# QuasarX1/astro-sph-tools

Hardware: AMD Instinct MI355X
Metric: Mpixels/s + particles/s, 10^8-particle 4096² projection at 1/2/4/8 MI355X (higher is better)
Workload: dtype f32; 1 GPU; cfg3: 1e+08 particles -> 4096^2 mass-weighted temperature map, wendland_c2, pixel-scale h, fp32; particles=100000000, grid=4096, kernel=wendland_c2, h_law=pixel, map=weighted, parallelism=single, accumulation=fp64, collective_overlap=False, streams=1, scatter_gate=False

## Files before the change

astro-sph-tools_amd/csrc/asp_device.hpp:

```cpp
#pragma once

#include <hip/hip_runtime.h>
#include <stdint.h>

namespace asp {

constexpr int kBlock = 256;
#ifndef ASP_DEP_BLOCK
#define ASP_DEP_BLOCK 512
#endif
constexpr int kDepBlock = ASP_DEP_BLOCK;
constexpr int kTile = 64;
constexpr int kTileShift = 6;
constexpr int kRow = kTile + 1;
constexpr int kTileWords = kTile * kRow;
constexpr int kWideTilesDefault = 256;
constexpr int kScaleBits = 49;
constexpr int kAccF64 = 0;
constexpr int kAccFix = 1;

struct Grid {
    double x_min, y_min;
    double psx;
    double psy_pix;
    double psy_cull;
    float xminf, yminf;
    float ipsx, ipsy;
    float mg;
    float mgl;
    int nx, ny, cs;
    int gnx;
    int ox;
    int ncx, ncy;
    int ntx, nty, ntiles;
    int nonsquare;
    int mixed;
    int wide_tiles;
    int gather_min;
    int gather_area;
};

struct Src64 {
    const double* u64;
    const double* v64;
    const double* cu64;
    const double* cv64;
    const double* h64;
    long long stride;
    const float* u32;
    const float* v32;
    const float* h32;
};

struct Box {
    int x0, x1, y0, y1;
};

struct Prep {
    float u, v, h;
    float lo;
    float hi;
    float hinv;
    float s0, s1;
    float thr;
    float band;
    int p;
    Box b;
};

struct Item {
    long long start;
    int tile;
    int count;
    int slab;
    int mode;
};

struct Merge {
    int tile;
    int slab0;
    int nslab;
    int pad;
};

__device__ __forceinline__ double corner_x(const Grid& g, int xi) {
    return g.x_min + (double)(xi + g.ox) * g.psx;
}
__device__ __forceinline__ double corner_y(const Grid& g, int yi) {
    return g.y_min + (double)yi * g.psy_pix;
}

__device__ __forceinline__ bool cull_pass(const Grid& g, double u, double v, double h,
                                          int xi, int yi) {
    xi += g.ox;
    int xi0 = (xi / g.cs) * g.cs, yi0 = (yi / g.cs) * g.cs;
    int xe = min(xi0 + g.cs, g.gnx), ye = min(yi0 + g.cs, g.ny);
    double h2 = 2.0 * h;
    double xlo = g.x_min + (double)xi0 * g.psx, xhi = g.x_min + (double)xe * g.psx;
    double ylo = g.y_min + (double)yi0 * g.psy_cull, yhi = g.y_min + (double)ye * g.psy_cull;
    return (u >= xlo - h2) && (u < xhi + h2) && (v >= ylo - h2) && (v < yhi + h2);
}

__device__ __forceinline__ void chunk_range(double w, double h, double w_min, double ps,
                                            int npx, int cs, int& c_lo, int& c_hi) {
    int nc = (npx + cs - 1) / cs;
    double h2 = 2.0 * h;
    c_lo = 0;
    c_hi = -1;
    if (!__builtin_isfinite(w) || !__builtin_isfinite(h)) return;
    auto lo_ok = [&](int c) { return w >= (w_min + (double)(c * cs) * ps) - h2; };
    auto hi_ok = [&](int c) {
        int e = min((c + 1) * cs, npx);
        return w < (w_min + (double)e * ps) + h2;
    };
    double est = floor((w + h2 - w_min) / ((double)cs * ps));
    int cmax = est < -1.0 ? -1 : (est > nc - 1.0 ? nc - 1 : (int)est);
    while (cmax >= 0 && !lo_ok(cmax)) --cmax;
    while (cmax + 1 <= nc - 1 && lo_ok(cmax + 1)) ++cmax;
    double est2 = ceil((w - h2 - w_min) / ((double)cs * ps)) - 1.0;
    int cmin = est2 < 0.0 ? 0 : (est2 > (double)nc ? nc : (int)est2);
    while (cmin <= nc - 1 && !hi_ok(cmin)) ++cmin;
    while (cmin - 1 >= 0 && hi_ok(cmin - 1)) --cmin;
    c_lo = cmin;
    c_hi = cmax;
}

struct Vals {
    double U, V, CU, CV, H;
};
__device__ __forceinline__ Vals src_values(const Grid& g, const Src64& s, int p) {
    Vals r;
    if (s.u64) {
        const long long o = (long long)p * s.stride;
        r.U = s.u64[o];
        r.V = s.v64[o];
        r.H = s.h64[p];
        r.CU = g.mixed ? s.cu64[o] : r.U;
        r.CV = g.mixed ? s.cv64[o] : r.V;
    } else {
        r.U = r.CU = s.u32[p];
        r.V = r.CV = s.v32[p];
        r.H = s.h32[p];
    }
    return r;
}
__device__ __forceinline__ double src_u(const Src64& s, int p, float u) {
    return s.u64 ? s.u64[(long long)p * s.stride] : (double)u;
}
__device__ __forceinline__ double src_v(const Src64& s, int p, float v) {
    return s.v64 ? s.v64[(long long)p * s.stride] : (double)v;
}

template <bool CULL = true>
__device__ __forceinline__ bool footprint(const Grid& g, const Src64& s, int p, float u, float v,
                                          float h, Box& b) {
    float hd = fabsf(2.0f * h);
    if (!(hd > 0.0f) || !__builtin_isfinite(hd)) {
        return false;
    }
    if (!__builtin_isfinite(u) || !__builtin_isfinite(v)) return false;
    float cx = (u - g.xminf) * g.ipsx, rx = hd * g.ipsx;
    float cy = (v - g.yminf) * g.ipsy, ry = hd * g.ipsy;
    float dx = (fabsf(u) + fabsf(g.xminf) + hd) * g.ipsx * 0x1p-20f + 0x1p-12f;
    float dy = (fabsf(v) + fabsf(g.yminf) + hd) * g.ipsy * 0x1p-20f + 0x1p-12f;
    float fx0 = fmaxf(ceilf(cx - rx - dx), (float)g.ox);
    float fx1 = fminf(floorf(cx + rx + dx), (float)(g.ox + g.nx - 1));
    float fy0 = fmaxf(ceilf(cy - ry - dy), 0.0f);
    float fy1 = fminf(floorf(cy + ry + dy), (float)(g.ny - 1));
    if (!(fx0 <= fx1) || !(fy0 <= fy1)) return false;
    b.x0 = (int)fx0 - g.ox;
    b.x1 = (int)fx1 - g.ox;
    b.y0 = (int)fy0;
    b.y1 = (int)fy1;
    if (CULL && (g.nonsquare || g.mixed)) {
        const Vals x = src_values(g, s, p);
        int c0, c1;
        chunk_range(x.CV, x.H, g.y_min, g.psy_cull, g.ny, g.cs, c0, c1);
        b.y0 = max(b.y0, c0 * g.cs);
        b.y1 = min(b.y1, min((c1 + 1) * g.cs, g.ny) - 1);
        if (b.y0 > b.y1) return false;
        if (g.mixed) {
            chunk_range(x.CU, x.H, g.x_min, g.psx, g.gnx, g.cs, c0, c1);
            b.x0 = max(b.x0, c0 * g.cs - g.ox);
            b.x1 = min(b.x1, min((c1 + 1) * g.cs, g.gnx) - 1 - g.ox);
            if (b.x0 > b.x1) return false;
        }
    }
    return true;
}

template <int KID>
__device__ __forceinline__ double kernel_norm64(float h) {
    double hd = (double)h;
    double h3 = hd * hd * hd;
    double r = __builtin_amdgcn_rcp(h3);
    r = r * (2.0 - h3 * r);
    if constexpr (KID == 0) return (1.0 / M_PI) * r;
    else if constexpr (KID == 1) return (21.0 / (16.0 * M_PI)) * r;
    else return 1.0;
}

template <int KID>
__device__ __forceinline__ double term_coef(float a, float h) {
    return (double)a * kernel_norm64<KID>(h);
}

template <int KID>
__device__ __forceinline__ float kernel_shape(float q) {
    if constexpr (KID == 0) {
        float q2 = q * q;
        float a = fmaf(q2, fmaf(0.75f, q, -1.5f), 1.0f);
        float t = 2.0f - q;
        float b = 0.25f * (t * t * t);
        return q < 1.0f ? a : (q < 2.0f ? b : 0.0f);
    } else if constexpr (KID == 1) {
        float t = fmaxf(fmaf(-0.5f, q, 1.0f), 0.0f);
        float t2 = t * t;
        return (t2 * t2) * fmaf(2.0f, q, 1.0f);
    } else {
        return 1.0f;
    }
}

__device__ __forceinline__ float rec_thr(float h) {
    float D = 2.0f * h;
    return D * D;
}
__device__ __forceinline__ float rec_band(float mg, float h) {
    float Da = fabsf(2.0f * h);
    float eps = 0x1p-21f * (mg + Da);
    float band = 4.0f * Da * eps + 2.0f * eps * eps + 0x1p-20f * Da * Da;
    if (h < 0.0f || !__builtin_isfinite(band)) band = __builtin_inff();
    return band;
}

__device__ __forceinline__ void set_band(Prep& P, float thr, float band) {
    P.lo = thr - band;
    P.hi = thr + band;
    P.thr = thr;
    P.band = band;
}

template <int KID, int ACC = kAccF64>
__device__ __forceinline__ bool prep_record(const Grid& g, const Src64& s, int p, float u,
                                            float v, float h, float a0, float a1, int k0,
                                            int k1, Prep& P) {
    if (!footprint(g, s, p, u, v, h, P.b)) return false;
    P.u = u;
    P.v = v;
    P.h = h;
    P.p = p;
    set_band(P, rec_thr(h), rec_band(g.mg, h));
    P.hinv = __builtin_amdgcn_rcpf(h);
    if constexpr (ACC == kAccFix) {
        P.s0 = (float)ldexp(term_coef<KID>(a0, h), k0);
        P.s1 = (float)ldexp(term_coef<KID>(a1, h), k1);
    } else {
        P.s0 = (float)term_coef<KID>(a0, h);
        P.s1 = (float)term_coef<KID>(a1, h);
    }
    return true;
}

__device__ __forceinline__ bool exact_pair(const Grid& g, const Src64& s, int p, int xi, int yi) {
    const Vals x = src_values(g, s, p);
    double dx = x.U - corner_x(g, xi);
    double dy = x.V - corner_y(g, yi);
    double r2 = dx * dx + dy * dy;
    double t = 2.0 * x.H;
    return (r2 < t * t) && cull_pass(g, x.CU, x.CV, x.H, xi, yi);
}

__device__ __forceinline__ bool decide(const Grid& g, const Src64& s, const Prep& P, int xi,
                                       int yi, float X, float Y, float& r2) {
    float dx = P.u - X;
    float dy = P.v - Y;
    r2 = dx * dx + dy * dy;
    bool in = r2 < P.lo;
    if (r2 >= P.lo && r2 <= P.hi) in = exact_pair(g, s, P.p, xi, yi);
    return in;
}

__device__ __forceinline__ unsigned long long f2fix(float f) {
    const double magic = 6755399441055744.0;
    return (unsigned long long)(__double_as_longlong((double)f + magic) -
                                __double_as_longlong(magic));
}

template <int ACC>
__device__ __forceinline__ void acc_add(unsigned long long* a, float t) {
    if constexpr (ACC == kAccFix)
        atomicAdd(a, f2fix(t));
    else
        atomicAdd((double*)a, (double)t);
}

template <int ACC>
__device__ __forceinline__ float acc_value(unsigned long long s, int k) {
    if constexpr (ACC == kAccFix)
        return (float)ldexp((double)(long long)s, -k);
    else
        return (float)__longlong_as_double((long long)s);
}

template <int ACC>
__device__ __forceinline__ unsigned long long acc_sum(unsigned long long a, unsigned long long b) {
    if constexpr (ACC == kAccFix)
        return a + b;
    else
        return (unsigned long long)__double_as_longlong(__longlong_as_double((long long)a) +
                                                        __longlong_as_double((long long)b));
}

__device__ __forceinline__ float bcast(float x, int lane) {
// ... 51 lines not shown
```

astro-sph-tools_amd/csrc/asp_project2d.hip:

```cpp
#include <hip/hip_runtime.h>

#include <algorithm>
#include <cmath>
#include <cstdint>
#include <cstdio>
#include <cstdlib>
#include <cstring>
#include <mutex>
#include <string>
#include <type_traits>
#include <vector>

#include "../../include/asp.h"
#include "asp_binning.hpp"
#include "asp_device.hpp"
#include "asp_host.hpp"

namespace asp {

constexpr int kCountBlock = 256;
#ifndef ASP_COUNT_UNROLL
#define ASP_COUNT_UNROLL 4
#endif
constexpr int kCountUnroll = ASP_COUNT_UNROLL;
// ... 697 lines not shown
    if (idx < 0) return;
    float4 r0, r1;
    load_rec(recs, start + idx, r0, r1);
    Prep P;
    rec_prep<ACC>(r0, r1, X0, Y0, kk, P);
    if constexpr (EXT) ext_coef(P, ext[start + idx], pass);
    small_box<KID, NOUT, ACC, 4>(g, s, P, P.b.x1 - P.b.x0 + 1, P.b.y1 - P.b.y0 + 1, X0, Y0, xt,
                                 yt, acc0, acc1);
}

constexpr int kGatherThreads = 64;
constexpr int kGatherRegions = 8;
constexpr int kGatherPix = 8 * kGatherThreads;
static_assert(kGatherRegions * kGatherPix == kTile * kTile, "8 regions x 512 pixels cover the tile");
constexpr int kKernelIndicator = ASP_KERNEL_INDICATOR;
struct GEntry {
    float u, v, lo, hi, hinv, s0, s1;
    int p;
    unsigned box;
};
constexpr unsigned kNoBox = 0x00ff00ffu;

template <int NOUT, int ACC>
struct GAcc {
    unsigned long long a0[8], a1[8];
    f2 p0[4], p1[4];
    double* t0;
    double* t1;
    __device__ __forceinline__ void init(double* tot) {
#pragma unroll
        for (int j = 0; j < 8; ++j) {
            a0[j] = 0;
            a1[j] = 0;
        }
#pragma unroll
        for (int k = 0; k < 4; ++k) {
            p0[k] = (f2){0.0f, 0.0f};
            p1[k] = (f2){0.0f, 0.0f};
        }
        t0 = tot + threadIdx.x;
        t1 = tot + kGatherPix + threadIdx.x;
        if constexpr (ACC != kAccFix) {
#pragma unroll
            for (int j = 0; j < 8; ++j) {
                t0[j * kGatherThreads] = 0.0;
                if (NOUT == 2) t1[j * kGatherThreads] = 0.0;
            }
        }
    }
    __device__ __forceinline__ void add(int j, float w, float s0, float s1) {
        if constexpr (ACC == kAccFix) {
            a0[j] += f2fix(s0 * w);
            if (NOUT == 2) a1[j] += f2fix(s1 * w);
        } else {
            p0[j >> 1][j & 1] = fmaf(s0, w, p0[j >> 1][j & 1]);
            if (NOUT == 2) p1[j >> 1][j & 1] = fmaf(s1, w, p1[j >> 1][j & 1]);
        }
    }
    __device__ __forceinline__ void add2(int k, f2 w, float s0, float s1) {
        if constexpr (ACC == kAccFix) {
            add(2 * k, w.x, s0, s1);
            add(2 * k + 1, w.y, s0, s1);
        } else {
            p0[k] = __builtin_elementwise_fma(w, (f2){s0, s0}, p0[k]);
            if (NOUT == 2) p1[k] = __builtin_elementwise_fma(w, (f2){s1, s1}, p1[k]);
        }
    }
    __device__ __forceinline__ void fold() {
        if constexpr (ACC != kAccFix) {
#pragma unroll
            for (int j = 0; j < 8; ++j) {
                t0[j * kGatherThreads] += (double)p0[j >> 1][j & 1];
                if (NOUT == 2) t1[j * kGatherThreads] += (double)p1[j >> 1][j & 1];
            }
#pragma unroll
            for (int k = 0; k < 4; ++k) {
                p0[k] = (f2){0.0f, 0.0f};
                p1[k] = (f2){0.0f, 0.0f};
            }
        }
    }
    __device__ __forceinline__ unsigned long long word0(int j) const {
        if constexpr (ACC == kAccFix) return a0[j];
        else return (unsigned long long)__double_as_longlong(t0[j * kGatherThreads]);
    }
    __device__ __forceinline__ unsigned long long word1(int j) const {
        if constexpr (ACC == kAccFix) return a1[j];
        else return (unsigned long long)__double_as_longlong(t1[j * kGatherThreads]);
    }
};

template <int NOUT, int ACC>
constexpr size_t gather_lds() {
    return ACC == kAccFix ? 8 : (size_t)NOUT * kGatherPix * 8;
}

struct GOwn {
    int r0, c0;
    int lr, lc;
    __device__ __forceinline__ int row(int j) const { return r0 + 8 * (j >> 2) + lr; }
    __device__ __forceinline__ int col(int j) const { return c0 + 8 * (j & 3) + lc; }
};
__device__ __forceinline__ GOwn gather_owner(int w) {
    const int lane = threadIdx.x;
    GOwn o;
    o.r0 = (w >> 1) * 16;
    o.c0 = (w & 1) * 32;
    o.lr = lane >> 3;
    o.lc = lane & 7;
    return o;
}

__device__ __forceinline__ float corner_off_x(const Grid& g, int k) { return (float)((double)k * g.psx); }
__device__ __forceinline__ float corner_off_y(const Grid& g, int k) { return (float)((double)k * g.psy_pix); }

struct GCorner {
    float X[2], Y[4];
    float xl[2], xh[2], yl[2], yh[2];
};
__device__ __forceinline__ GCorner gather_corners(const Grid& g, const GOwn& o) {
    GCorner c;
    c.X[0] = corner_off_x(g, o.row(0));
    c.X[1] = corner_off_x(g, o.row(4));
#pragma unroll
    for (int k = 0; k < 4; ++k) c.Y[k] = corner_off_y(g, o.col(k));
#pragma unroll
    for (int r = 0; r < 2; ++r) {
        c.xl[r] = corner_off_x(g, o.r0 + 8 * r);
        c.xh[r] = corner_off_x(g, o.r0 + 8 * r + 7);
        c.yl[r] = corner_off_y(g, o.c0 + 16 * r);
        c.yh[r] = corner_off_y(g, o.c0 + 16 * r + 15);
    }
    return c;
}

__device__ __forceinline__ unsigned edge_mask(const GCorner& c, float u, float v, float thr) {
    float dx2[2], dy2[2];
#pragma unroll
    for (int r = 0; r < 2; ++r) {
        const float dx = u - fminf(fmaxf(u, c.xl[r]), c.xh[r]);
        const float dy = v - fminf(fmaxf(v, c.yl[r]), c.yh[r]);
        dx2[r] = dx * dx;
        dy2[r] = dy * dy;
    }
    const float lim = thr * (1.0f + 0x1p-8f);
    unsigned m = 0u;
#pragma unroll
    for (int r = 0; r < 2; ++r)
#pragma unroll
        for (int k = 0; k < 2; ++k) m |= (dx2[r] + dy2[k] < lim) ? 1u << (2 * r + k) : 0u;
    return m;
}

__device__ __forceinline__ GEntry make_gentry(const Prep& P, int X0, int Y0, float scale) {
    GEntry e;
    e.u = P.u; e.v = P.v; e.lo = P.lo; e.hi = P.hi; e.hinv = P.hinv;
    e.s0 = P.s0 * scale; e.s1 = P.s1 * scale; e.p = P.p;
    e.box = (unsigned)(P.b.x0 - X0) | ((unsigned)(P.b.x1 - X0) << 8) |
            ((unsigned)(P.b.y0 - Y0) << 16) | ((unsigned)(P.b.y1 - Y0) << 24);
    return e;
}

__device__ __forceinline__ bool meets_region(unsigned box, const GOwn& o) {
    return (int)(box & 255u) <= o.r0 + 15 && (int)((box >> 8) & 255u) >= o.r0 &&
           (int)((box >> 16) & 255u) <= o.c0 + 31 && (int)(box >> 24) >= o.c0;
}

__device__ __forceinline__ GEntry lane_entry(const GEntry& e, int l) {
    GEntry E;
    E.u = bcast(e.u, l); E.v = bcast(e.v, l); E.lo = bcast(e.lo, l); E.hi = bcast(e.hi, l);
    E.hinv = bcast(e.hinv, l); E.s0 = bcast(e.s0, l); E.s1 = bcast(e.s1, l);
    E.p = bcast(e.p, l); E.box = (unsigned)bcast((int)e.box, l);
    return E;
}

__device__ __forceinline__ unsigned block_hits(unsigned box, const GOwn& o) {
    const int x0 = box & 255u, x1 = (box >> 8) & 255u;
    const int y0 = (box >> 16) & 255u, y1 = box >> 24;
    unsigned m = 0u;
#pragma unroll
    for (int j = 0; j < 8; ++j) {
        const int br = o.r0 + 8 * (j >> 2), bc = o.c0 + 8 * (j & 3);
        if (x0 <= br + 7 && x1 >= br && y0 <= bc + 7 && y1 >= bc) m |= 1u << j;
    }
    return m;
}


template <int KID, int NOUT, int ACC>
__device__ __forceinline__ void gather_entry(const Grid& g, const Src64& s, const GEntry& E,
                                             int X0, int Y0, const GOwn& o, const GCorner& c,
                                             GAcc<NOUT, ACC>& ga) {
    const unsigned m = block_hits(E.box, o);
    const int x0 = E.box & 255u, x1 = (E.box >> 8) & 255u;
    const int y0 = (E.box >> 16) & 255u, y1 = E.box >> 24;
    unsigned in = 0u, amb = 0u;
#pragma unroll
    for (int j = 0; j < 8; ++j) {
        if (m & (1u << j)) {
            const float dx = E.u - c.X[j >> 2], dy = E.v - c.Y[j & 3];
            const float r2 = dx * dx + dy * dy;
            const bool inb = (unsigned)(o.row(j) - x0) <= (unsigned)(x1 - x0) &&
                             (unsigned)(o.col(j) - y0) <= (unsigned)(y1 - y0);
            in |= (inb && r2 < E.lo) ? (1u << j) : 0u;
            amb |= (inb && r2 >= E.lo && r2 <= E.hi) ? (1u << j) : 0u;
        }
    }
    for (unsigned a = amb; a; a &= a - 1u) {
        const int j = __builtin_ctz(a);
        if (exact_pair(g, s, E.p, X0 + o.row(j), Y0 + o.col(j))) in |= 1u << j;
    }
    const float sc = 1.0f / kShapeScale<KID>;
#pragma unroll
    for (int j = 0; j < 8; ++j) {
        if (in & (1u << j)) {
            const float dx = E.u - c.X[j >> 2], dy = E.v - c.Y[j & 3];
            const float r2 = dx * dx + dy * dy;
            const float wk = kernel_shape<KID>(__builtin_amdgcn_sqrtf(r2) * E.hinv) * sc;
            ga.add(j, wk, E.s0, E.s1);
        }
    }
}

template <int KID, int NOUT, int ACC>
__device__ __forceinline__ void gather_entry_masked(float u, float vs, float hinv, float s0,
                                                    float s1, float nt2, unsigned bm,
                                                    const GCorner& c, GAcc<NOUT, ACC>& ga) {
    const f2 hv = {-hinv, -hinv};
    const f2 dead = {nt2, nt2};
    const f2 vv = {vs, vs};
#pragma unroll
    for (int r = 0; r < 2; ++r) {
        if (bm & (3u << (2 * r))) {
            const float dxs = (u - c.X[r]) * hinv;
            const f2 dx2 = {dxs * dxs, dxs * dxs};
#pragma unroll
            for (int k = 0; k < 2; ++k) {
                if (bm & (1u << (2 * r + k))) {
                    const f2 dys = __builtin_elementwise_fma(hv, (f2){c.Y[2 * k], c.Y[2 * k + 1]}, vv);
                    const f2 r2 = __builtin_elementwise_fma(dys, dys, dx2);
                    f2 q;
                    q.x = __builtin_amdgcn_sqrtf(r2.x);
                    q.y = __builtin_amdgcn_sqrtf(r2.y);
                    ga.add2(2 * r + k, edge_shape2<KID, true>(q, dead), s0, s1);
                }
            }
        }
    }
}

template <int KID, int NOUT, int ACC>
__device__ __forceinline__ void gather_walk(const Grid& g, const Src64& s, const GEntry& mine,
                                            int X0, int Y0, const GOwn& o, const GCorner& c,
                                            GAcc<NOUT, ACC>& ga) {
    if (KID != kKernelIndicator && !g.nonsquare && !g.mixed) {
        const unsigned em = mine.box == kNoBox ? 0u : edge_mask(c, mine.u, mine.v, mine.hi);
        const float vs = mine.v * mine.hinv;
        const unsigned emd = em | (__float_as_uint(edge_dead2(mine.lo, mine.hi)) & ~15u);
        unsigned long long m = __ballot(em != 0u);
        while (m) {
            const int l = __builtin_ctzll(m);
            m &= m - 1;
            const unsigned w = (unsigned)bcast((int)emd, l);
            gather_entry_masked<KID, NOUT, ACC>(bcast(mine.u, l), bcast(vs, l), bcast(mine.hinv, l),
                                                bcast(mine.s0, l), bcast(mine.s1, l),
                                                __uint_as_float(w), w & 15u, c, ga);
        }
    } else {
        unsigned long long m = __ballot(meets_region(mine.box, o));
        while (m) {
            const int l = __builtin_ctzll(m);
            m &= m - 1;
            gather_entry<KID, NOUT, ACC>(g, s, lane_entry(mine, l), X0, Y0, o, c, ga);
        }
    }
    ga.fold();
}

template <int NOUT, int ACC>
__device__ __forceinline__ void gather_emit(const Grid& g, const GAcc<NOUT, ACC>& ga,
                                            const GOwn& o, int X0, int Y0, int slab,
                                            unsigned long long* slabs, int k0, int k1,
                                            float* out0, float* out1, int flags) {
    if (slab >= 0) {
        unsigned long long* dst = slabs + (long long)slab * NOUT * kTilePix;
#pragma unroll
        for (int j = 0; j < 8; ++j) {
            const int k = o.row(j) * kTile + o.col(j);
            dst[k] = ga.word0(j);
            if (NOUT == 2) dst[kTilePix + k] = ga.word1(j);
        }
        return;
    }
    const int TW = min(kTile, g.nx - X0), TH = min(kTile, g.ny - Y0);
#pragma unroll
    for (int j = 0; j < 8; ++j) {
        if (o.row(j) >= TW || o.col(j) >= TH) continue;
        const long long off = (long long)(X0 + o.row(j)) * g.ny + (Y0 + o.col(j));
        emit_pixel<NOUT, ACC>(off, ga.word0(j), NOUT == 2 ? ga.word1(j) : 0ull, k0, k1, out0,
                              out1, flags);
    }
}

__device__ __forceinline__ bool is_small(int bw, int bh) { return bw <= 4 && bh <= 4; }

template <int NOUT>
constexpr size_t deposit_lds() {
    return (size_t)NOUT * kTileWords * 8 + 2 * kTile * 4;
}

template <int KID, int NOUT, int ACC, int EXT = 0>
__global__ __launch_bounds__(kDepBlock) __attribute__((amdgpu_waves_per_eu(4))) void k_deposit(
    Grid g, Src64 s, const float4* __restrict__ recs, const Item* __restrict__ items,
    const int* __restrict__ order, const int2* __restrict__ tile_k,
    unsigned long long* __restrict__ slabs, float* __restrict__ out0, float* __restrict__ out1,
    int flags, const float4* __restrict__ ext, int pass) {
    extern __shared__ __attribute__((aligned(16))) unsigned long long acc[];
    unsigned long long* acc0 = acc;
    unsigned long long* acc1 = acc + kTileWords;
    float* xt = (float*)(acc + NOUT * kTileWords);
    float* yt = xt + kTile;
    __shared__ int defer_lds[kDepBlock / 64][kDeferCap];
    const Item it = items[order[blockIdx.x]];
    if (it.mode != 0) return;
    int tx = it.tile / g.nty, ty = it.tile - (it.tile / g.nty) * g.nty;
    int X0 = tx * kTile, Y0 = ty * kTile;
    int TW = min(kTile, g.nx - X0), TH = min(kTile, g.ny - Y0);
    if (it.count == 0) {
        if (flags & kFlagAccumulate) return;
        for (int k = threadIdx.x; k < kTilePix; k += kDepBlock) {
            int lx = k >> kTileShift, ly = k & (kTile - 1);
            if (lx >= TW || ly >= TH) continue;
            long long o = (long long)(X0 + lx) * g.ny + (Y0 + ly);
            out0[o] = 0.0f;
            if (NOUT == 2) out1[o] = 0.0f;
        }
        return;
    }
    const int2 kk = ACC == kAccFix ? tile_k[it.tile] : make_int2(0, 0);
    tile_prologue<NOUT, kDepBlock>(g, X0, Y0, acc, xt, yt);
    const int lane = threadIdx.x & 63;
    const Corner3 c3 = corner3(g);
    int* dlist = defer_lds[threadIdx.x >> 6];
    int ndef = 0;
    auto batch = [&](int i, const float4& r0, const float4& r1, const float4& e) {
        Prep P;
        P.b = Box{0, -1, 0, -1};
        bool live = i < it.count;
        if (live) {
            rec_prep<ACC>(r0, r1, X0, Y0, kk, P);
            if constexpr (EXT) ext_coef(P, e, pass);
        }
        live = live && P.b.x0 <= P.b.x1;
        const int bw = P.b.x1 - P.b.x0 + 1, bh = P.b.y1 - P.b.y0 + 1;
        const bool small = live && is_small(bw, bh);
        bool amb = false;
        if (small) {
            if (bw <= 3 && bh <= 3)
                amb = !small3_fast<KID, NOUT, ACC>(P, bw, bh, X0, Y0, c3, acc0, acc1);
            else
                amb = true;
        }
        {
            unsigned long long am = __ballot(amb);
            if (am) {
                if (amb) dlist[ndef + __popcll(am & ((1ull << lane) - 1ull))] = i;
                ndef += __popcll(am);
                if (ndef >= 64) {
                    ndef -= 64;
                    deferred<KID, NOUT, ACC, EXT>(g, s, recs, ext, pass, it.start, dlist, ndef,
                                                  64, X0, Y0, kk, xt, yt, acc0, acc1, lane);
                }
            }
        }
        unsigned long long mid = __ballot(live && !small);
        while (mid) {
            int l = __builtin_ctzll(mid);
            mid &= mid - 1;
            Prep Q = bcast_prep(P, l);
            sweep<KID, NOUT, ACC>(g, s, Q, X0, Y0, xt, yt, acc0, acc1, lane);
        }
    };
    const int last = it.count - 1;
    float4 r0, r1, q0, q1, re, qe;
    auto load_ext = [&](long long i, float4& e) {
        if constexpr (EXT) e = ext[i];
        else e = make_float4(0.0f, 0.0f, 0.0f, 0.0f);
    };
    load_rec(recs, it.start + min((int)threadIdx.x, last), r0, r1);
    load_ext(it.start + min((int)threadIdx.x, last), re);
    load_rec(recs, it.start + min((int)threadIdx.x + kDepBlock, last), q0, q1);
    load_ext(it.start + min((int)threadIdx.x + kDepBlock, last), qe);
    for (int base = 0; base < it.count; base += kDepBlock) {
        float4 n0, n1, ne;
        load_rec(recs, it.start + min(base + (int)threadIdx.x + 2 * kDepBlock, last), n0, n1);
        load_ext(it.start + min(base + (int)threadIdx.x + 2 * kDepBlock, last), ne);
        batch(base + threadIdx.x, r0, r1, re);
        r0 = q0;
        r1 = q1;
        re = qe;
        q0 = n0;
        q1 = n1;
        qe = ne;
    }
    if (ndef > 0)
        deferred<KID, NOUT, ACC, EXT>(g, s, recs, ext, pass, it.start, dlist, 0, ndef, X0, Y0, kk,
                                      xt, yt, acc0, acc1, lane);
    __syncthreads();
    if (it.slab >= 0) {
        unsigned long long* dst = slabs + (long long)it.slab * NOUT * kTilePix;
        for (int k = threadIdx.x; k < kTilePix; k += kDepBlock) {
            const int w = pix(k >> kTileShift, k & (kTile - 1));
            dst[k] = acc0[w];
            if (NOUT == 2) dst[kTilePix + k] = acc1[w];
        }
        return;
    }
    for (int k = threadIdx.x; k < kTilePix; k += kDepBlock) {
        int lx2 = k >> kTileShift, ly = k & (kTile - 1);
        if (lx2 >= TW || ly >= TH) continue;
        long long o = (long long)(X0 + lx2) * g.ny + (Y0 + ly);
        const int w = pix(lx2, ly);
        emit_pixel<NOUT, ACC>(o, acc0[w], NOUT == 2 ? acc1[w] : 0ull, kk.x, kk.y, out0, out1,
                              flags);
    }
}

template <int KID, int NOUT, int ACC, int EXT = 0>
__global__ __launch_bounds__(kGatherThreads) void k_gather(
    Grid g, Src64 s, const float4* __restrict__ recs, const Item* __restrict__ items,
    const int* __restrict__ order, const int2* __restrict__ tile_k,
    unsigned long long* __restrict__ slabs, float* __restrict__ out0, float* __restrict__ out1,
    int flags, const float4* __restrict__ ext, int pass) {
    extern __shared__ __attribute__((aligned(16))) double tot[];
    const Item it = items[order[blockIdx.x / kGatherRegions]];
    if (it.mode != 1) return;
    const int tx = it.tile / g.nty, ty = it.tile - (it.tile / g.nty) * g.nty;
    const int X0 = tx * kTile, Y0 = ty * kTile;
    const int2 kk = ACC == kAccFix ? tile_k[it.tile] : make_int2(0, 0);
    const int lane = threadIdx.x;
    const int last = it.count - 1;
    float4 r0, r1, e = make_float4(0.0f, 0.0f, 0.0f, 0.0f);
    load_rec(recs, it.start + min(lane, last), r0, r1);
    if constexpr (EXT) e = ext[it.start + min(lane, last)];
    const GOwn o = gather_owner(blockIdx.x % kGatherRegions);
    GAcc<NOUT, ACC> ga;
    ga.init(tot);
    const GCorner cc = gather_corners(g, o);
    for (int base = 0; base < it.count; base += 64) {
        GEntry mine;
        mine.box = kNoBox;
        if (base + lane < it.count) {
            Prep P;
            rec_prep<ACC>(r0, r1, X0, Y0, kk, P);
            if constexpr (EXT) ext_coef(P, e, pass);
            P.u += corner_off_x(g, P.b.x0 - X0);
            P.v += corner_off_y(g, P.b.y0 - Y0);
            mine = make_gentry(P, X0, Y0, kShapeScale<KID>);
        }
        load_rec(recs, it.start + min(base + 64 + lane, last), r0, r1);
        if constexpr (EXT) e = ext[it.start + min(base + 64 + lane, last)];
        gather_walk<KID, NOUT, ACC>(g, s, mine, X0, Y0, o, cc, ga);
    }
    gather_emit<NOUT, ACC>(g, ga, o, X0, Y0, it.slab, slabs, kk.x, kk.y, out0, out1, flags);
}

constexpr int kMergeBatch = 8;
template <int NOUT, int ACC>
__global__ __launch_bounds__(kBlock) void k_merge(Grid g, const Merge* __restrict__ merges,
                                                  const unsigned long long* __restrict__ slabs,
                                                  const int2* __restrict__ tile_k,
                                                  float* __restrict__ out0,
                                                  float* __restrict__ out1, int flags) {
    const Merge m = merges[blockIdx.x];
    int tx = m.tile / g.nty, ty = m.tile - (m.tile / g.nty) * g.nty;
    int X0 = tx * kTile, Y0 = ty * kTile;
    int TW = min(kTile, g.nx - X0), TH = min(kTile, g.ny - Y0);
    const int k = blockIdx.y * kBlock + threadIdx.x;
    int lx = k >> kTileShift, ly = k & (kTile - 1);
    if (lx >= TW || ly >= TH) return;
    const int2 kk = ACC == kAccFix ? tile_k[m.tile] : make_int2(0, 0);
    const unsigned long long* src = slabs + (long long)m.slab0 * NOUT * kTilePix + k;
    unsigned long long s0 = 0, s1 = 0;
    int j = 0;
    for (; j + kMergeBatch <= m.nslab; j += kMergeBatch) {
        unsigned long long b0[kMergeBatch], b1[kMergeBatch];
#pragma unroll
        for (int q = 0; q < kMergeBatch; ++q) {
            const unsigned long long* p = src + (long long)(j + q) * NOUT * kTilePix;
            b0[q] = p[0];
            b1[q] = NOUT == 2 ? p[kTilePix] : 0ull;
        }
#pragma unroll
        for (int q = 0; q < kMergeBatch; ++q) {
            s0 = acc_sum<ACC>(s0, b0[q]);
            if (NOUT == 2) s1 = acc_sum<ACC>(s1, b1[q]);
        }
    }
    for (; j < m.nslab; ++j) {
        const unsigned long long* p = src + (long long)j * NOUT * kTilePix;
        s0 = acc_sum<ACC>(s0, p[0]);
        if (NOUT == 2) s1 = acc_sum<ACC>(s1, p[kTilePix]);
    }
    long long o = (long long)(X0 + lx) * g.ny + (Y0 + ly);
    emit_pixel<NOUT, ACC>(o, s0, s1, kk.x, kk.y, out0, out1, flags);
}

template <int KID, int NOUT, int ACC>
__global__ __launch_bounds__(kGatherThreads) void k_wide(
    Grid g, Src64 s, const float* __restrict__ u, const float* __restrict__ v,
    const float* __restrict__ h, const float* __restrict__ a0, const float* __restrict__ a1,
    const int* __restrict__ wide_list, int n_wide, const int* __restrict__ ctr,
    float* __restrict__ out0, float* __restrict__ out1) {
    extern __shared__ __attribute__((aligned(16))) double tot[];
    const int t = blockIdx.x / kGatherRegions;
    const int tx = t / g.nty, ty = t - (t / g.nty) * g.nty;
    const int X0 = tx * kTile, Y0 = ty * kTile;
    const int TW = min(kTile, g.nx - X0), TH = min(kTile, g.ny - Y0);
    const int k0 = ACC == kAccFix ? scale_exp(n_wide, __uint_as_float((unsigned)ctr[cWideMax0])) : 0;
    const int k1 = (ACC == kAccFix && NOUT == 2)
                       ? scale_exp(n_wide, __uint_as_float((unsigned)ctr[cWideMax1])) : 0;
    const int lane = threadIdx.x;
    const GOwn o = gather_owner(blockIdx.x % kGatherRegions);
    GAcc<NOUT, ACC> ga;
    ga.init(tot);
    const GCorner cc = gather_corners(g, o);
    bool any = false;
    for (int c = 0; c < n_wide; c += 64) {
        GEntry mine;
        mine.box = kNoBox;
        const int k = c + lane;
        if (k < n_wide) {
            const int p = wide_list[k];
            Prep P;
            if (prep_record<KID, ACC>(g, s, p, u[p], v[p], h[p], a0[p], NOUT == 2 ? a1[p] : 0.0f,
                                      k0, k1, P) &&
                clip(P.b, X0, Y0, TW, TH)) {
                P.u = (float)(src_u(s, p, P.u) - corner_x(g, X0));
                P.v = (float)(src_v(s, p, P.v) - corner_y(g, Y0));
                set_band(P, rec_thr(P.h), rec_band(g.mgl, P.h));
                mine = make_gentry(P, X0, Y0, kShapeScale<KID>);
            }
        }
        any = any || __ballot(mine.box != kNoBox) != 0ull;
        gather_walk<KID, NOUT, ACC>(g, s, mine, X0, Y0, o, cc, ga);
    }
    if (!any) return;
    gather_emit<NOUT, ACC>(g, ga, o, X0, Y0, -1, nullptr, k0, k1, out0, out1, kFlagAccumulate);
}

__device__ __forceinline__ long long gather_slots(const Grid& g, int kid, unsigned box, float u,
                                                  float v, float hi) {
    const int x0 = box & 255u, x1 = (box >> 8) & 255u, y0 = (box >> 16) & 255u, y1 = box >> 24;
    const bool edge = kid != kKernelIndicator && !g.nonsquare && !g.mixed;
    long long c = 0;
    for (int w = 0; w < kGatherRegions; ++w) {
        const int r0 = (w >> 1) * 16, c0 = (w & 1) * 32;
        if (edge) {
            GOwn o;
            o.r0 = r0;
            o.c0 = c0;
            o.lr = o.lc = 0;
            c += 128LL * __builtin_popcount(edge_mask(gather_corners(g, o), u, v, hi));
            continue;
        }
        for (int r = 0; r < 2; ++r) {
            const int br = r0 + 8 * r;
            if (!(x0 <= br + 7 && x1 >= br)) continue;
            {
                for (int k = 0; k < 4; ++k) {
                    const int bc = c0 + 8 * k;
                    if (y0 <= bc + 7 && y1 >= bc) c += 64;
                }
            }
        }
    }
    return c;
}

__global__ __launch_bounds__(kBlock) void k_evals(Grid g, int kid, Src64 s,
                                                  const float4* __restrict__ recs,
                                                  const Item* __restrict__ items, int n_items,
                                                  const float* __restrict__ u,
                                                  const float* __restrict__ v,
                                                  const float* __restrict__ h,
                                                  const int* __restrict__ wide_list, int n_wide,
                                                  unsigned long long* __restrict__ evals) {
    long long c0 = 0, c1 = 0, c2 = 0;
    if ((int)blockIdx.x < n_items) {
        const Item it = items[blockIdx.x];
        const int tx = it.tile / g.nty, ty = it.tile - (it.tile / g.nty) * g.nty;
        const int X0 = tx * kTile, Y0 = ty * kTile;
        for (int i = threadIdx.x; i < it.count; i += kBlock) {
            float4 r0, r1;
            load_rec(recs, it.start + i, r0, r1);
            Prep P;
            rec_prep<kAccF64>(r0, r1, X0, Y0, make_int2(0, 0), P);
            const int bw = P.b.x1 - P.b.x0 + 1, bh = P.b.y1 - P.b.y0 + 1;
            if (bw <= 0) continue;
            if (it.mode == 1) {
                c1 += gather_slots(g, kid, __float_as_uint(r1.w),
                                   P.u + corner_off_x(g, P.b.x0 - X0),
                                   P.v + corner_off_y(g, P.b.y0 - Y0), P.hi);
            } else if (bw <= 3 && bh <= 3) {
                c0 += 9;
            } else if (is_small(bw, bh)) {
                c0 += bw * bh;
            } else {
                const int passes = bh <= 64 ? (bw + 64 / bh - 1) / (64 / bh) : bw * ((bh + 63) / 64);
                c0 += 64LL * passes;
            }
        }
    } else {
        const int t = blockIdx.x - n_items;
        const int tx = t / g.nty, ty = t - (t / g.nty) * g.nty;
        const int X0 = tx * kTile, Y0 = ty * kTile;
        const int TW = min(kTile, g.nx - X0), TH = min(kTile, g.ny - Y0);
        for (int i = threadIdx.x; i < n_wide; i += kBlock) {
            const int p = wide_list[i];
            Prep P;
            if (prep_record<2>(g, s, p, u[p], v[p], h[p], 0.0f, 0.0f, 0, 0, P) &&
                clip(P.b, X0, Y0, TW, TH)) {
                const unsigned box = (unsigned)(P.b.x0 - X0) | ((unsigned)(P.b.x1 - X0) << 8) |
                                     ((unsigned)(P.b.y0 - Y0) << 16) | ((unsigned)(P.b.y1 - Y0) << 24);
                set_band(P, rec_thr(P.h), rec_band(g.mgl, P.h));
                c2 += gather_slots(g, kid, box, (float)(src_u(s, p, P.u) - corner_x(g, X0)),
                                   (float)(src_v(s, p, P.v) - corner_y(g, Y0)), P.hi);
            }
        }
    }
    if (c0) atomicAdd(&evals[0], (unsigned long long)c0);
    if (c1) atomicAdd(&evals[1], (unsigned long long)c1);
    if (c2) atomicAdd(&evals[2], (unsigned long long)c2);
}

__global__ __launch_bounds__(kBlock) void k_ratio(float* __restrict__ out0,
                                                  const float* __restrict__ out1, long long m) {
    long long i = (long long)blockIdx.x * kBlock + threadIdx.x;
    long long stride = (long long)gridDim.x * kBlock;
    for (; i < m; i += stride) {
        float d = out1[i];
        out0[i] = d != 0.0f ? out0[i] / d : 0.0f;
    }
}

constexpr int kPairsBlock = 256;
template <int MODE>
__global__ __launch_bounds__(kPairsBlock) void k_pairs(
    Grid g, Src64 s, const float4* __restrict__ recs, const long long* __restrict__ tile_start,
    const int* __restrict__ tile_total, const int* __restrict__ wide_list, int n_wide,
    const float* __restrict__ u, const float* __restrict__ v, const float* __restrict__ h,
    int t0, int* __restrict__ pixcnt, long long* __restrict__ tile_pairs,
    const long long* __restrict__ tile_base, long long* __restrict__ offsets,
    int* __restrict__ particle, double* __restrict__ r2out, int* __restrict__ overflow) {
    __shared__ int cur[kTilePix];
    __shared__ float xt[kTile], yt[kTile];
    __shared__ long long wsum[kPairsBlock / 64];
    __shared__ long long soff[MODE == 1 ? kTilePix + 1 : 1];
    const int t = t0 + blockIdx.x;
    const int tx = t / g.nty, ty = t - (t / g.nty) * g.nty;
    const int X0 = tx * kTile, Y0 = ty * kTile;
    const int TW = min(kTile, g.nx - X0), TH = min(kTile, g.ny - Y0);
    const int lane = threadIdx.x & 63, wv = threadIdx.x >> 6;
    constexpr int kPer = kTilePix / kPairsBlock;
    long long* off = offsets + (long long)blockIdx.x * kTilePix;
    if constexpr (MODE == 1) {
        const int* c = pixcnt + (long long)t * kTilePix + threadIdx.x * kPer;
        long long loc[kPer], run = 0;
#pragma unroll
        for (int k = 0; k < kPer; ++k) {
            loc[k] = run;
            run += c[k];
        }
        long long x = run;
#pragma unroll
        for (int o = 1; o < 64; o <<= 1) {
            long long y = __shfl_up(x, o);
            if (lane >= o) x += y;
        }
        if (lane == 63) wsum[wv] = x;
        __syncthreads();
        long long base = tile_base[blockIdx.x] + x - run;
        for (int k = 0; k < wv; ++k) base += wsum[k];
#pragma unroll
        for (int k = 0; k < kPer; ++k) {
            soff[threadIdx.x * kPer + k] = base + loc[k];
            off[threadIdx.x * kPer + k] = base + loc[k];
        }
        if (threadIdx.x == kPairsBlock - 1) {
            soff[kTilePix] = base + run;
            off[kTilePix] = base + run;
        }
    }
    for (int k = threadIdx.x; k < kTilePix; k += kPairsBlock) cur[k] = 0;
    corner_tables(g, X0, Y0, xt, yt);
    __syncthreads();
    auto emit_box = [&](const Prep& P) {
        for (int xi = P.b.x0; xi <= P.b.x1; ++xi)
            for (int yi = P.b.y0; yi <= P.b.y1; ++yi) {
                float r2f;
                if (!decide(g, s, P, xi, yi, xt[xi - P.b.x0], yt[yi - P.b.y0], r2f)) continue;
                const int lp = (xi - X0) * kTile + (yi - Y0);
                const int k = atomicAdd(&cur[lp], 1);
                if constexpr (MODE == 1) {
                    const long long slot = soff[lp] + k;
                    if (slot >= soff[lp + 1]) {
// ... 1508 lines not shown
```

Baseline: 5273 Mpixels/s.

## Reorder deposit particles per wave to spread LDS bank pairs

```diff
diff --git a/astro-sph-tools_amd/csrc/asp_device.hpp b/astro-sph-tools_amd/csrc/asp_device.hpp
--- a/astro-sph-tools_amd/csrc/asp_device.hpp
+++ b/astro-sph-tools_amd/csrc/asp_device.hpp
@@ -10,6 +10,9 @@
 #define ASP_DEP_BLOCK 512
 #endif
 constexpr int kDepBlock = ASP_DEP_BLOCK;
+#ifndef ASP_DEP_ORDER
+#define ASP_DEP_ORDER 1
+#endif
 constexpr int kTile = 64;
 constexpr int kTileShift = 6;
 constexpr int kRow = kTile + 1;
diff --git a/astro-sph-tools_amd/csrc/asp_project2d.hip b/astro-sph-tools_amd/csrc/asp_project2d.hip
--- a/astro-sph-tools_amd/csrc/asp_project2d.hip
+++ b/astro-sph-tools_amd/csrc/asp_project2d.hip
@@ -1023,6 +1023,77 @@
     }
 }
 
+constexpr int kPoolBatches = 2;
+constexpr int kPool = 64 * kPoolBatches;
+static_assert(kRow % 16 == 1, "bank pair of pix(x, y) is (x + y) mod 16");
+struct OrderLds {
+    int cnt[16];
+    unsigned lvl[64];
+    unsigned char tab[kPool];
+};
+
+__device__ __forceinline__ void wave_lds_sync() {
+    __builtin_amdgcn_fence(__ATOMIC_RELEASE, "wavefront");
+    __builtin_amdgcn_wave_barrier();
+    __builtin_amdgcn_fence(__ATOMIC_ACQUIRE, "wavefront");
+}
+
+__device__ __forceinline__ unsigned order_pool(const unsigned (&key)[kPoolBatches], int n,
+                                               OrderLds& w, int lane) {
+    if (lane < 16) w.cnt[lane] = 0;
+    wave_lds_sync();
+    int bank[kPoolBatches], r[kPoolBatches];
+    bool big = false;
+#pragma unroll
+    for (int j = 0; j < kPoolBatches; ++j) {
+        bank[j] = (int)(((key[j] & 255u) + ((key[j] >> 16) & 255u)) & 15u);
+        r[j] = j * 64 + lane < n ? atomicAdd(&w.cnt[bank[j]], 1) : 0;
+        big |= r[j] >= 64;
+    }
+    wave_lds_sync();
+    const int c = w.cnt[lane & 15];
+    {
+        int T = 0;
+        unsigned m = 0;
+#pragma unroll
+        for (int b = 0; b < 16; ++b) {
+            const int cb = __builtin_amdgcn_readlane(c, b);
+            T += min(cb, lane);
+            m |= cb > lane ? 1u << b : 0u;
+        }
+        w.lvl[lane] = (unsigned)T << 16 | m;
+    }
+    wave_lds_sync();
+    int pos[kPoolBatches];
+    if (__ballot(big)) {
+#pragma unroll
+        for (int j = 0; j < kPoolBatches; ++j) {
+            int p = 0;
+            for (int b = 0; b < 16; ++b) {
+                const int cb = __builtin_amdgcn_readlane(c, b);
+                p += min(cb, r[j]) + (b < bank[j] && cb > r[j] ? 1 : 0);
+            }
+            pos[j] = p;
+        }
+    } else {
+#pragma unroll
+        for (int j = 0; j < kPoolBatches; ++j) {
+            const unsigned e = w.lvl[r[j]];
+            pos[j] = (int)(e >> 16) + __popc(e & ((1u << bank[j]) - 1u));
+        }
+    }
+#pragma unroll
+    for (int j = 0; j < kPoolBatches; ++j)
+        if (j * 64 + lane < n)
+            w.tab[(pos[j] & 63) * kPoolBatches + (pos[j] >> 6)] = (unsigned char)(j * 64 + lane);
+    wave_lds_sync();
+    unsigned idx = 0u;
+#pragma unroll
+    for (int j = 0; j < kPoolBatches; ++j) idx |= (unsigned)w.tab[lane * kPoolBatches + j] << (8 * j);
+    wave_lds_sync();
+    return idx;
+}
+
 __device__ __forceinline__ bool is_small(int bw, int bh) { return bw <= 4 && bh <= 4; }
 
 template <int NOUT>
@@ -1042,6 +1113,8 @@
     float* xt = (float*)(acc + NOUT * kTileWords);
     float* yt = xt + kTile;
     __shared__ int defer_lds[kDepBlock / 64][kDeferCap];
+    constexpr bool kOrdered = ASP_DEP_ORDER && NOUT == 2;
+    __shared__ OrderLds order_lds[kOrdered ? kDepBlock / 64 : 1];
     const Item it = items[order[blockIdx.x]];
     if (it.mode != 0) return;
     int tx = it.tile / g.nty, ty = it.tile - (it.tile / g.nty) * g.nty;
@@ -1108,21 +1181,68 @@
         if constexpr (EXT) e = ext[i];
         else e = make_float4(0.0f, 0.0f, 0.0f, 0.0f);
     };
-    load_rec(recs, it.start + min((int)threadIdx.x, last), r0, r1);
-    load_ext(it.start + min((int)threadIdx.x, last), re);
-    load_rec(recs, it.start + min((int)threadIdx.x + kDepBlock, last), q0, q1);
-    load_ext(it.start + min((int)threadIdx.x + kDepBlock, last), qe);
-    for (int base = 0; base < it.count; base += kDepBlock) {
-        float4 n0, n1, ne;
-        load_rec(recs, it.start + min(base + (int)threadIdx.x + 2 * kDepBlock, last), n0, n1);
-        load_ext(it.start + min(base + (int)threadIdx.x + 2 * kDepBlock, last), ne);
-        batch(base + threadIdx.x, r0, r1, re);
-        r0 = q0;
-        r1 = q1;
-        re = qe;
-        q0 = n0;
-        q1 = n1;
-        qe = ne;
+    if constexpr (kOrdered) {
+        OrderLds& ol = order_lds[threadIdx.x >> 6];
+        constexpr int kWaves = kDepBlock / 64;
+        auto pstart = [&](int k) { return (max(k, 0) * kWaves + (int)(threadIdx.x >> 6)) * kPool; };
+        auto pcount = [&](int k) { return k < 0 ? 0 : max(0, min(kPool, it.count - pstart(k))); };
+        auto load_keys = [&](int k, unsigned (&key)[kPoolBatches]) {
+#pragma unroll
+            for (int j = 0; j < kPoolBatches; ++j)
+                key[j] = __float_as_uint(
+                    ((const float*)recs)[(it.start + min(pstart(k) + j * 64 + lane, last)) * 8 + 7]);
+        };
+        unsigned key[kPoolBatches];
+        load_keys(0, key);
+        asm volatile("" ::: "memory");
+        load_rec(recs, it.start + min(pstart(0), last), r0, r1);
+        load_ext(it.start + min(pstart(0), last), re);
+        load_rec(recs, it.start + min(pstart(0) + 1, last), q0, q1);
+        load_ext(it.start + min(pstart(0) + 1, last), qe);
+        unsigned cidx = 0u;
+#pragma nounroll
+        for (int k = -1; k * (kWaves * kPool) < it.count; ++k) {
+            const int n = pcount(k), nn = pcount(k + 1);
+            const unsigned nidx = nn > 0 ? order_pool(key, nn, ol, lane) : 0u;
+            load_keys(k + 2, key);
+#pragma unroll
+            for (int j = 0; j < kPoolBatches; ++j) {
+                constexpr int kAhead = 2;
+                const int ni = j + kAhead < kPoolBatches
+                    ? pstart(k) + (int)(cidx >> (8 * ((j + kAhead) % kPoolBatches)) & 255u)
+                    : pstart(k + 1) + (int)(nidx >> (8 * ((j + kAhead) % kPoolBatches)) & 255u);
+                float4 n0, n1, ne;
+                load_rec(recs, it.start + min(ni, last), n0, n1);
+                load_ext(it.start + min(ni, last), ne);
+                batch(j * 64 + lane < n ? pstart(k) + (int)(cidx >> (8 * j) & 255u) : it.count, r0, r1,
+                      re);
+                r0 = q0;
+                r1 = q1;
+                re = qe;
+                q0 = n0;
+                q1 = n1;
+                qe = ne;
+            }
+            cidx = nidx;
+        }
+        static_assert(kPoolBatches >= 2, "a batch is loaded two batches ahead: at most one pool");
+    } else {
+        load_rec(recs, it.start + min((int)threadIdx.x, last), r0, r1);
+        load_ext(it.start + min((int)threadIdx.x, last), re);
+        load_rec(recs, it.start + min((int)threadIdx.x + kDepBlock, last), q0, q1);
+        load_ext(it.start + min((int)threadIdx.x + kDepBlock, last), qe);
+        for (int base = 0; base < it.count; base += kDepBlock) {
+            float4 n0, n1, ne;
+            load_rec(recs, it.start + min(base + (int)threadIdx.x + 2 * kDepBlock, last), n0, n1);
+            load_ext(it.start + min(base + (int)threadIdx.x + 2 * kDepBlock, last), ne);
+            batch(base + threadIdx.x, r0, r1, re);
+            r0 = q0;
+            r1 = q1;
+            re = qe;
+            q0 = n0;
+            q1 = n1;
+            qe = ne;
+        }
     }
     if (ndef > 0)
         deferred<KID, NOUT, ACC, EXT>(g, s, recs, ext, pass, it.start, dlist, 0, ndef, X0, Y0, kk,
```

Measured after the change: 5437 Mpixels/s (median of 6 runs). +3.1%, better.
